# NVlabs/neuralrgbd

Hardware: AMD Instinct MI355X
Metric: depth frames/sec @256x192x64cand, 5-view window; warp-kernel HBM GB/s vs peak (higher is better)
Workload: dtype f32; 1 GPU; plane-sweep grid 256x192x64cand (image 1024x768); config_id=B, depth_candidates=64, views=5, streams_per_gpu=1, streams_total=1, parallelism=replicas x1 (independent video streams)

## Files before the change

### include/nrgbd.h

```cpp
#ifndef NRGBD_H
#define NRGBD_H

#ifdef __cplusplus
extern "C" {
#endif

#define NRGBD_OK             0
#define NRGBD_E_NULL        -1
#define NRGBD_E_SHAPE       -2
#define NRGBD_E_ALIGN       -3
#define NRGBD_E_ARG         -4

#define NRGBD_DIST_L2        0
#define NRGBD_DIST_L1        1

#define NRGBD_MAX_D        256
#define NRGBD_MAX_V         16

#define NRGBD_INTERFACE_VERSION "0.10"
const char* nrgbd_version(void);
const char* nrgbd_strerror(int code);

int nrgbd_homography_terms(const float* K, const float* R, long r_view_stride, long r_row_stride,
                           const float* t, long t_view_stride, long t_elem_stride, float* KR, float* Kt,
// ... 167 lines not shown
int nrgbd_conv_wino_dw4_workspace(int N, int H, int W, int Cout, size_t* bytes);
int nrgbd_conv_wino_dw4_f32(const float* x, const float* x_ss, int x_relu, float x_unit, const float* w_wino, float* y, float* stats,
                            void* workspace, size_t workspace_bytes, int N, int H, int W, int Cin, int Cout, void* stream);
int nrgbd_conv_wino_dw_unit_f32(const float* x, const float* x_ss, float x_unit, const float* w_wino, float* y, float* stats,
                                int N, int H, int W, int Cin, int Cout, void* stream);

int nrgbd_conv2d_rnet_f32(const float* x, const float* w_packed, const float* bias, int out_lrelu, float* y,
                          int ldy, int ycoff, int cout_valid, int mode, int pa, int pb,
                          int N, int H, int W, int Cin, int Cout, void* stream);
int nrgbd_rnet_pack(const float* dpv_log, const float* feat, int feat_planar, float* out, int D, int Cf, long P,
                    void* stream);

int nrgbd_conv2d_taps_f32(const float* x, const float* x_ss, int x_relu, const float* w_packed, float* y, float* stats,
                          int N, int H, int W, int Cin, int Cout, int taps, int in_stride, void* stream);
int nrgbd_space_to_depth2(const float* x, int nchw, float* y, int N, int C, int H, int W, int Cp, void* stream);
int nrgbd_conv2d_wgrad_workgroups(int N, int H, int W, int Cin, int Cout);
int nrgbd_conv2d_wgrad_f32(const float* x, const float* gy, float* partial, float* dw, int N, int H, int W, int Cin, int Cout,
                           int dilation, void* stream);
int nrgbd_conv2d_workgroups(int N, int H, int W);
int nrgbd_conv_pack_weights(const float* w, float* w_packed, int Cin, int Cout, int taps, void* stream);
int nrgbd_conv2d_3x3_f32(const float* x, const float* x_ss, int x_relu,
                         const float* res, const float* res_ss, int res_relu,
                         float* materialized, const float* w_packed, const float* bias, int out_lrelu,
                         float* y, float* stats, int N, int H, int W, int Cin, int Cout, int dilation,
                         void* stream);
int nrgbd_bn_finalize(const float* stats, int num_workgroups, int C, long count,
                      const float* gamma, const float* beta, float eps, float momentum,
                      float* running_mean, float* running_var, float* scale_shift, unsigned int* collapse_count, long long* batches_tracked, void* stream);
int nrgbd_bn_small_stats(int nseg, const float* const* x, const long* rows, int C, const float* const* gamma, const float* const* beta,
                     const float* eps, const float* momentum, float* const* running_mean, float* const* running_var,
// ... 62 lines not shown
```

### neuralrgbd_amd/_lib.py

```python
import ctypes
import os

_HERE = os.path.dirname(os.path.abspath(__file__))
LIB_PATH = os.path.join(_HERE, "csrc", "libnrgbd_hip.so")

_c = ctypes
_P = _c.c_void_p
_F = _c.c_float
_I = _c.c_int
_L = _c.c_long
_D = _c.c_double
_Z = _c.c_size_t

GATHER_MAX_V = 6
DEPTH_MAX_THRESHOLDS = 512
DEPTH_EVAL_MAX_SETS = 8
DGF_TILE = (16, 64)


class WindowSlots(ctypes.Structure):
    _fields_ = [("idx", _I * (GATHER_MAX_V + 1))]


SIGNATURES = {
# ... 59 lines not shown
    "nrgbd_conv3d_wgrad_ranges": (_I, []),
    "nrgbd_conv3d_wgrad_f32": (_I, [_P, _P, _P, _P, _I, _I, _I, _I, _P]),
    "nrgbd_bn3d_finalize": (_I, [_P, _I, _L, _P, _P, _F, _F, _P, _P, _P, _P, _P, _P]),
    "nrgbd_bn2d_partial_floats": (_I, [_I]),
    "nrgbd_bn2d_train_act": (_I, [_P, _P, _P, _F, _I, _P, _P, _P, _P, _I, _I, _L, _P]),
    "nrgbd_avgpool8": (_I, [_P, _P, _I, _I, _I, _P]),
    "nrgbd_conv2d_few_f32": (_I, [_P, _I, _P, _P, _I, _P, _I, _I, _I, _I, _I, _I, _I, _P]),
    "nrgbd_avgpool_cl": (_I, [_P, _P, _I, _I, _I, _I, _I, _P]),
    "nrgbd_scatter_channels": (_I, [_P, _L, _L, _L, _I, _I, _I, _P, _I, _I, _I, _L, _P]),
    "nrgbd_bias_act_nchw": (_I, [_P, _P, _F, _I, _I, _L, _P]),
    "nrgbd_conv2d_workgroups": (_I, [_I, _I, _I]),
    "nrgbd_conv2d_wgrad_workgroups": (_I, [_I, _I, _I, _I, _I]),
    "nrgbd_conv2d_wgrad_f32": (_I, [_P, _P, _P, _P, _I, _I, _I, _I, _I, _I, _P]),
    "nrgbd_conv2d_taps_f32": (_I, [_P, _P, _I, _P, _P, _P, _I, _I, _I, _I, _I, _I, _I, _P]),
    "nrgbd_space_to_depth2": (_I, [_P, _I, _P, _I, _I, _I, _I, _I, _P]),
    "nrgbd_conv_pack_weights": (_I, [_P, _P, _I, _I, _I, _P]),
    "nrgbd_conv2d_3x3_f32": (_I, [_P, _P, _I, _P, _P, _I, _P, _P, _P, _I, _P, _P, _I, _I, _I, _I, _I, _I, _P]),
    "nrgbd_conv2d_rnet_f32": (_I, [_P, _P, _P, _I, _P, _I, _I, _I, _I, _I, _I, _I, _I, _I, _I, _I, _P]),
    "nrgbd_rnet_pack": (_I, [_P, _P, _I, _P, _I, _I, _L, _P]),
    "nrgbd_bn_finalize": (_I, [_P, _I, _I, _L, _P, _P, _F, _F, _P, _P, _P, _P, _P, _P]),
    "nrgbd_logsoftmax_rows": (_I, [_P, _P, _L, _I, _P]),
    "nrgbd_logsoftmax_d_bwd": (_I, [_P, _P, _F, _P, _I, _L, _P]),
    "nrgbd_logsoftmax_rows_bwd": (_I, [_P, _P, _P, _L, _I, _P]),
    "nrgbd_nll_workgroups": (_I, [_L]),
    "nrgbd_nll_fwd": (_I, [_P, _P, _L, _I, _L, _I, _P, _P, _P]),
    "nrgbd_nll_bwd": (_I, [_P, _L, _P, _P, _P, _I, _L, _I, _P]),
    "nrgbd_adam_step": (_I, [_P, _P, _P, _P, _P, _P, _I, _D, _D, _D, _D, _D, _I, _P]),
    "nrgbd_grad_norm_workspace": (_L, [_P, _I]),
    "nrgbd_grad_norm": (_I, [_P, _P, _I, _D, _P, _Z, _P, _P, _P]),
    "nrgbd_scale_tensors": (_I, [_P, _P, _I, _P, _P]),
# ... 51 lines not shown
```

### neuralrgbd_amd/csrc/conv2d.hip

```cpp
#include <cstdlib>

#include "conv_tile.hpp"

namespace nrgbd {

constexpr int kT2 = 16;

struct Conv2dArgs {
    const float* x;
    const float* x_ss;
    const float* res;
    const float* res_ss;
    float* mat;
    const float* wp;
    const float* bias;
    float* y;
    float* stats;
    int x_relu, res_relu, out_lrelu;
    int N, H, W, Cin;
    int xcd;
    int ldy;
    int ycoff;
    int cout_valid;
    int up;
// ... 247 lines not shown
        }
        if (khalf == 0) {
#pragma unroll
            for (int f = 0; f < NF; ++f) {
                red[wv * (2 * COUT) + f * 32 + i] = s1[f];
                red[wv * (2 * COUT) + COUT + f * 32 + i] = s2[f];
            }
        }
        __syncthreads();
        if (tid < 2 * COUT)
            a.stats[(size_t)tile_id * (2 * COUT) + tid] =
                (red[tid] + red[2 * COUT + tid]) + (red[4 * COUT + tid] + red[6 * COUT + tid]);
    }
}

__global__ void conv_pack_weights_kernel(const float* __restrict__ w, float* __restrict__ wp, int Cin, int Cout, int taps) {
    const int ncblk = Cin / kCB, G4 = kCB / 8, nf = Cout / 32;
    const long total = (long)taps * Cin * Cout;
    const long idx = (long)blockIdx.x * 256 + threadIdx.x;
    if (idx >= total) return;
    long t = idx;
    const int e = t & 3; t >>= 2;
    const int ln = t & 63; t >>= 6;
    const int nfrag = t % nf; t /= nf;
    const int g = t % G4; t /= G4;
    const int cblk = t % ncblk; const int tap = (int)(t / ncblk);
    const int cout = nfrag * 32 + (ln & 31);
    const int cin = cblk * kCB + (ln >> 5) * (kCB / 2) + g * 4 + e;
    wp[idx] = w[((size_t)cout * Cin + cin) * taps + tap];
}
// ... 37 lines not shown
        v.x = __builtin_fmaf(v.x, ss[0], ss[1]); v.y = __builtin_fmaf(v.y, ss[2], ss[3]);
        v.z = __builtin_fmaf(v.z, ss[4], ss[5]); v.w = __builtin_fmaf(v.w, ss[6], ss[7]);
    }
    if (x_relu) { v.x = fmaxf(v.x, 0.f); v.y = fmaxf(v.y, 0.f); v.z = fmaxf(v.z, 0.f); v.w = fmaxf(v.w, 0.f); }
    if (res) {
        f32x4 r = *reinterpret_cast<const f32x4*>(res + p * C + c);
        if (res_ss) {
            const float* ss = res_ss + 2 * c;
            r.x = __builtin_fmaf(r.x, ss[0], ss[1]); r.y = __builtin_fmaf(r.y, ss[2], ss[3]);
            r.z = __builtin_fmaf(r.z, ss[4], ss[5]); r.w = __builtin_fmaf(r.w, ss[6], ss[7]);
        }
        if (res_relu) { r.x = fmaxf(r.x, 0.f); r.y = fmaxf(r.y, 0.f); r.z = fmaxf(r.z, 0.f); r.w = fmaxf(r.w, 0.f); }
        v = v + r;
    }
    *reinterpret_cast<f32x4*>(y + p * ldy + c) = v;
}

__global__ __launch_bounds__(256) void bn_finalize_kernel(const float* __restrict__ stats, int nwg, int C, double count,
                                                          const float* __restrict__ gamma, const float* __restrict__ beta,
                                                          float eps, float momentum, float* __restrict__ running_mean,
                                                          float* __restrict__ running_var, float* __restrict__ ss, unsigned int* __restrict__ collapse_count, long long* __restrict__ batches_tracked) {
    __shared__ double sh[2][256];
    const int c = blockIdx.x, tid = threadIdx.x;
    double s1 = 0.0, s2 = 0.0;
    for (int g = tid; g < nwg; g += 256) {
        s1 += (double)stats[(size_t)g * 2 * C + c];
        s2 += (double)stats[(size_t)g * 2 * C + C + c];
    }
    sh[0][tid] = s1; sh[1][tid] = s2;
    __syncthreads();
// ... 123 lines not shown
    if ((long)N * H * W * Cin * in_stride * in_stride >= (1L << 32)) return NRGBD_E_SHAPE;
    Conv2dArgs a{x, x_ss, nullptr, nullptr, nullptr, w_packed, nullptr, y, stats, x_relu, 0, 0, N, H, W, Cin,
                 0, Cout, 0, Cout, 0, 0, 0, nullptr, in_stride};
    const int nwg = ceil_div(W, kT2) * ceil_div(H, kT2) * N;
    hipStream_t st = (hipStream_t)stream;
    if (taps == 1) {
        if (Cout == 32) launch_conv2d_taps<32, 1>(a, nwg, st);
        else if (Cout == 64) launch_conv2d_taps<64, 1>(a, nwg, st);
        else if (Cout == 128) launch_conv2d_taps<128, 1>(a, nwg, st);
        else return NRGBD_E_SHAPE;
    } else {
        if (Cout == 32) launch_conv2d_taps<32, 4>(a, nwg, st);
        else if (Cout == 64) launch_conv2d_taps<64, 4>(a, nwg, st);
        else return NRGBD_E_SHAPE;
    }
    NRGBD_CHECK_LAUNCH();
    return NRGBD_OK;
}

extern "C" int nrgbd_conv2d_workgroups(int N, int H, int W) {
    using namespace nrgbd;
    if (N <= 0 || H <= 0 || W <= 0) return NRGBD_E_SHAPE;
    return ceil_div(W, kT2) * ceil_div(H, kT2) * N;
}

extern "C" int nrgbd_conv_pack_weights(const float* w, float* wp, int Cin, int Cout, int taps, void* stream) {
    using namespace nrgbd;
    if (!w || !wp) return NRGBD_E_NULL;
    if (Cin <= 0 || Cin % kCB || Cout <= 0 || Cout % 32 || (taps != 9 && taps != 27 && taps != 4 && taps != 1)) return NRGBD_E_SHAPE;
    const long total = (long)taps * Cin * Cout;
// ... 112 lines not shown
    return NRGBD_OK;
}

extern "C" int nrgbd_nhwc_act(const float* x, const float* x_ss, int x_relu, const float* res, const float* res_ss,
                              int res_relu, float* y, long P, int C, int ldy, void* stream) {
    using namespace nrgbd;
    if (!x || !y) return NRGBD_E_NULL;
    if (P <= 0 || C < 4 || (C & 3) || ldy < C || (ldy & 3)) return NRGBD_E_SHAPE;
    const long total = P * (C >> 2);
    hipLaunchKernelGGL(nhwc_act_kernel, dim3((unsigned)((total + 255) / 256)), dim3(256), 0, (hipStream_t)stream, x, x_ss,
                       x_relu, res, res_ss, res_relu, y, P, C, ldy);
    NRGBD_CHECK_LAUNCH();
    return NRGBD_OK;
}

extern "C" int nrgbd_bn_finalize(const float* stats, int num_workgroups, int C, long count, const float* gamma,
                                 const float* beta, float eps, float momentum, float* running_mean, float* running_var,
                                 float* scale_shift, unsigned int* collapse_count, long long* batches_tracked, void* stream) {
    using namespace nrgbd;
    if (!stats || !gamma || !beta || !scale_shift) return NRGBD_E_NULL;
    if (num_workgroups <= 0 || count <= 0 || C <= 0) return NRGBD_E_SHAPE;
    if ((running_mean == nullptr) != (running_var == nullptr)) return NRGBD_E_NULL;
    hipLaunchKernelGGL(bn_finalize_kernel, dim3(C), dim3(256), 0, (hipStream_t)stream, stats, num_workgroups, C,
                       (double)count, gamma, beta, eps, momentum, running_mean, running_var, scale_shift, collapse_count, batches_tracked);
    NRGBD_CHECK_LAUNCH();
    return NRGBD_OK;
}
```

### neuralrgbd_amd/csrc/warpvol.hip

```cpp
#include "common.hpp"

namespace nrgbd {

struct WarpVolArgs {
    const float* src; long sv, sc, sy, sx;
    const float* ref; long rc, ry, rx;
    const float* KR; const float* Kt; const float* rays; const float* d_candi;
    const float* bv_cur; const float* bv_pred;
    float* out;
    float cx, cy;
    int align, V, Cs, D, h, w;
    int channels_last;
    int ld;
};

__global__ __launch_bounds__(256) void warp_volume_kernel(const WarpVolArgs a) {
    const size_t hw = (size_t)a.h * a.w;
    const size_t p = (size_t)blockIdx.x * 256 + threadIdx.x;
    const int k = blockIdx.y;
    if (p >= hw) return;
    const int y = (int)(p / a.w), x = (int)(p - (size_t)y * a.w);
    const float rx = a.rays[p], ry = a.rays[hw + p], rz = a.rays[2 * hw + p];
    const float d = a.d_candi[k];
    const float wf = (float)a.w, hf = (float)a.h;
// ... 14 lines not shown
            o[(size_t)(v * a.Cs + c) * plane] = lerp4(pl[onw], pl[one], pl[osw], pl[ose], b);
        }
    }
    int ch = a.V * a.Cs;
    if (a.ref) {
        for (int c = 0; c < a.Cs; ++c) o[(size_t)(ch + c) * plane] = a.ref[c * a.rc + y * a.ry + x * a.rx];
        ch += a.Cs;
    }
    if (a.bv_cur) o[(size_t)ch * plane] = a.bv_cur[(size_t)k * hw + p] - a.bv_pred[(size_t)k * hw + p];
    if (a.channels_last)
        for (int c = n_ch; c < ld; ++c) o[c] = 0.f;
}

template <bool ALIGN>
__global__ __launch_bounds__(256) void warp_volume_cl16_kernel(const WarpVolArgs a, float rcx, float rcy) {
    const size_t hw = (size_t)a.h * a.w;
    const size_t p = (size_t)blockIdx.x * 256 + threadIdx.x;
    const int k = blockIdx.y;
    if (p >= hw) return;
    const int y = (int)(p / a.w), x = (int)(p - (size_t)y * a.w);
    const float rx = a.rays[p], ry = a.rays[hw + p], rz = a.rays[2 * hw + p];
    const float d = a.d_candi[k];
    const float wf = (float)a.w, hf = (float)a.h;
    float o[16];
#pragma unroll
    for (int v = 0; v < 4; ++v) {
        const SweepTerm st = make_sweep_term(a.KR + 9 * v, a.Kt + 3 * v, rx, ry, rz);
        float ix, iy;
        sweep_sample_pos_fast<ALIGN>(st, d, a.cx, a.cy, rcx, rcy, wf, hf, ix, iy);
        const Bilinear b = bilinear_zeros(ix, iy, a.w, a.h);
        const float* s = a.src + v * a.sv;
        const float4 A = *reinterpret_cast<const float4*>(s + b.y0 * a.sy + b.x0 * a.sx);
        const float4 B = *reinterpret_cast<const float4*>(s + b.y0 * a.sy + b.x1 * a.sx);
        const float4 C = *reinterpret_cast<const float4*>(s + b.y1 * a.sy + b.x0 * a.sx);
        const float4 Dd = *reinterpret_cast<const float4*>(s + b.y1 * a.sy + b.x1 * a.sx);
        o[3 * v + 0] = lerp4(A.x, B.x, C.x, Dd.x, b);
        o[3 * v + 1] = lerp4(A.y, B.y, C.y, Dd.y, b);
        o[3 * v + 2] = lerp4(A.z, B.z, C.z, Dd.z, b);
    }
    const float4 r = *reinterpret_cast<const float4*>(a.ref + y * a.ry + x * a.rx);
    o[12] = r.x; o[13] = r.y; o[14] = r.z;
    o[15] = a.bv_cur[(size_t)k * hw + p] - a.bv_pred[(size_t)k * hw + p];
    float4* dst = reinterpret_cast<float4*>(a.out + ((size_t)k * hw + p) * 16);
#pragma unroll
    for (int q = 0; q < 4; ++q) dst[q] = make_float4(o[4 * q], o[4 * q + 1], o[4 * q + 2], o[4 * q + 3]);
}

template <int V, int CP, bool ALIGN>
__global__ __launch_bounds__(256) void warp_volume_cl_kernel(const WarpVolArgs a, float rcx, float rcy) {
    constexpr int C = 3 * V + 4;
    static_assert(CP % 4 == 0 && CP >= C, "padded voxel holds the assembly in whole 16-byte words");
    const size_t hw = (size_t)a.h * a.w;
    const size_t p = (size_t)blockIdx.x * 256 + threadIdx.x;
    const int k = blockIdx.y;
    if (p >= hw) return;
    const int y = (int)(p / a.w), x = (int)(p - (size_t)y * a.w);
    const float rx = a.rays[p], ry = a.rays[hw + p], rz = a.rays[2 * hw + p];
    const float d = a.d_candi[k];
    const float wf = (float)a.w, hf = (float)a.h;
    float o[CP];
// ... 86 lines not shown
```

### neuralrgbd_amd/nets.py

```python
import math

import numpy as np
import torch
import torch.nn as nn
import torch.nn.functional as F


def _conv_bn2d(cin, cout, k, stride, pad, dilation, track=False):
    p = dilation if dilation > 1 else pad
    return nn.Sequential(
        nn.Conv2d(cin, cout, k, stride=stride, padding=p, dilation=dilation, bias=False),
        nn.BatchNorm2d(cout, track_running_stats=track),
    )


def _conv_bn3d(cin, cout):
    return nn.Sequential(nn.Conv3d(cin, cout, 3, stride=1, padding=1, bias=False), nn.BatchNorm3d(cout))


def _conv_lrelu(cin, cout):
    return nn.Sequential(nn.Conv2d(cin, cout, 3, stride=1, padding=1, bias=True), nn.LeakyReLU())


def _deconv_lrelu(cin, cout):
# ... 5 lines not shown
        if isinstance(m, (nn.Conv2d, nn.Conv3d)):
            fan = int(np.prod(m.kernel_size)) * m.out_channels
            m.weight.data.normal_(0, math.sqrt(2.0 / fan))
        elif isinstance(m, (nn.BatchNorm2d, nn.BatchNorm3d)):
            m.weight.data.fill_(1)
            m.bias.data.zero_()



def _no_kernel(what):
    from ._lib import NrgbdError
    return NrgbdError("no hand-written kernel for " + what)


class _Act(object):
    __slots__ = ("z", "ss", "relu", "r", "r_ss", "r_relu")

    def __init__(self, z, ss=None, relu=False, r=None, r_ss=None, r_relu=False):
        self.z, self.ss, self.relu, self.r, self.r_ss, self.r_relu = z, ss, relu, r, r_ss, r_relu


_PACKERS = {
    "taps": lambda ops, w: ops.conv_pack_weights(w),
    "s2": lambda ops, w: ops.conv_s2_pack(w),
    "pc": lambda ops, w: ops.conv_wino_pack32(w) if w.shape[0] == 32 and w.dim() == 4 else ops.conv_wino_pack(w),
    "dw": lambda ops, w: ops.conv_wino_dw_pack(w),
    "dw4": lambda ops, w: ops.conv_wino_dw4_pack(w),
    "direct": lambda ops, w: ops.conv3d_pack_weights(w),
    "cout1": lambda ops, w: w[0].reshape(w.shape[1], 27).t().contiguous(),
}


def padded_channels(c):
    return -(-int(c) // 16) * 16


def pad_input_channels(w, cin):
    if cin == w.shape[1]:
        return w
    return torch.cat((w, w.new_zeros((w.shape[0], cin - w.shape[1]) + tuple(w.shape[2:]))), dim=1)


def _packed(owner, conv, kind, mult=1.0, cin=None):
    from . import ops
    cache = owner.__dict__.setdefault("_wp_cache", {})
# ... 214 lines not shown
                and ops.conv_wino_supported(a.z.shape[0], a.z.shape[1], a.z.shape[2], conv.in_channels, conv.out_channels, 1))
        if wino:
            z, st, mat = ops.conv_wino(a.z, _packed(self, conv, "pc"), conv.out_channels, 1, d, x_ss=a.ss, x_relu=a.relu,
                                       res=a.r, res_ss=a.r_ss, res_relu=a.r_relu, materialize=materialize,
                                       want_stats=_needs_stats(bn))
        elif mfma:
            z, st, mat = ops.conv2d(a.z, _packed(self, conv, "taps"), conv.out_channels, d, x_ss=a.ss, x_relu=a.relu,
                                    res=a.r, res_ss=a.r_ss, res_relu=a.r_relu, materialize=materialize,
                                    want_stats=_needs_stats(bn))
        else:
            mat = a.z if (a.ss is None and a.r is None and not a.relu) else \
                ops.nhwc_act(a.z, a.ss, a.relu, a.r, a.r_ss, a.r_relu)
            s2 = (conv.kernel_size == (3, 3) and conv.stride == (2, 2) and conv.padding == (1, 1) and d == 1
                  and mat.shape[1] % 2 == 0 and mat.shape[2] % 2 == 0 and conv.out_channels in (32, 64))
            if s2:
                z, st = ops.conv2d_taps(ops.space_to_depth2(mat), _packed(self, conv, "s2"), conv.out_channels, 4,
                                        want_stats=_needs_stats(bn))
            else:
                raise _no_kernel("feature CNN layer %d -> %d, kernel %s, stride %s, dilation %d on a %d x %d map" % (
                    conv.in_channels, conv.out_channels, tuple(conv.kernel_size), tuple(conv.stride), d, mat.shape[1], mat.shape[2]))
        count = z.shape[0] * z.shape[1] * z.shape[2]
        return _Act(z, _bn_scale_shift(bn, st, count, "cm" if wino else "rows"), relu), mat

    def _pointwise_cl(self, conv, m, stride=1, want_stats=False):
        from . import ops
        N, H, W, C = m.shape
        if C % 16 != 0 or conv.out_channels not in (32, 64, 128) or H % stride or W % stride:
            raise _no_kernel("1x1 layer %d -> %d, stride %d on a %d x %d map" % (C, conv.out_channels, stride, H, W))
        return ops.conv2d_taps(m.contiguous(), _packed(self, conv, "taps"), conv.out_channels, 1, want_stats=want_stats, stride=stride)

    def _pointwise_bn_cl(self, seq, m, stride=1):
        conv, bn = seq[0], seq[1]
        z, st = self._pointwise_cl(conv, m, stride, want_stats=_needs_stats(bn))
        return _Act(z, _bn_scale_shift(bn, st, z.shape[0] * z.shape[1] * z.shape[2]), False)

    def _block_cl(self, blk, a):
        y1, m = self._conv_bn_cl(blk.conv1[0], a, relu=True, materialize=True)
        y2, _ = self._conv_bn_cl(blk.conv2, y1, relu=False)
        if blk.downsample is None:
            return _Act(y2.z, y2.ss, False, r=m)
        sk = self._pointwise_bn_cl(blk.downsample, m, blk.downsample[0].stride[0])
        return _Act(y2.z, y2.ss, False, r=sk.z, r_ss=sk.ss)

    def fused_ok(self, x):
        return x.is_cuda and not torch.is_grad_enabled() and x.dtype == torch.float32

    def forward_channels_last(self, x):
        from . import ops
        conv, bn = self.firstconv[0]
        if x.shape[2] % 4 or x.shape[3] % 4:
            raise _no_kernel("image %d x %d: the plane-sweep grid is the image / 4 (models/basic.py:254-263), both sides must be multiples of 4"
                             % (x.shape[2], x.shape[3]))
        z, st = ops.conv2d_taps(ops.space_to_depth2(x.contiguous(), nchw=True), _packed(self, conv, "s2"), conv.out_channels, 4,
                                want_stats=_needs_stats(bn))
        a = _Act(z, _bn_scale_shift(bn, st, z.numel() // z.shape[-1]), True)
        for i in (2, 4):
            a, _ = self._conv_bn_cl(self.firstconv[i], a, relu=True)
        for blk in self.layer1:
            a = self._block_cl(blk, a)
        half = ops.nhwc_act(a.z, a.ss, a.relu, a.r, a.r_ss, a.r_relu)
        a = _Act(half)
        for blk in self.layer2:
            a = self._block_cl(blk, a)
        quarter = None
        for k, blk in enumerate(self.layer3):
            y1, m = self._conv_bn_cl(blk.conv1[0], a, relu=True, materialize=True)
            if k == 0:
                quarter = m
            y2, _ = self._conv_bn_cl(blk.conv2, y1, relu=False)
            if blk.downsample is None:
                a = _Act(y2.z, y2.ss, False, r=m)
            else:
                sk = self._pointwise_bn_cl(blk.downsample, m, blk.downsample[0].stride[0])
                a = _Act(y2.z, y2.ss, False, r=sk.z, r_ss=sk.ss)
        for blk in self.layer4:
            a = self._block_cl(blk, a)
# ... 8 lines not shown
            pools = {8: p8, 16: p16, 32: p32, 64: ops.avgpool_cl(p32, 2)}
        else:
            pools = {k: ops.avgpool_cl(deep, k) for k in self.SPP_WINDOWS}
        zs, norms = [], []
        for i in (4, 3, 2, 1):
            branch = getattr(self, "branch%d" % i)
            z, _ = self._pointwise_cl(branch[1][0], pools[self.SPP_WINDOWS[i - 1]])
            zs.append(z)
            norms.append(branch[1][1])
        sss = _bn_scale_shift_small(norms, zs)
        cat = ops.spp_concat(quarter, deep, list(zip(zs, sss)))
        y, _ = self._conv_bn_cl(self.lastconv[0], _Act(cat), relu=True)
        head = self.lastconv[2]
        if head.out_channels not in (32, 64, 128):
            raise _no_kernel("feature_dim %d (1x1 head): 32, 64 or 128" % head.out_channels)
        feat, _ = ops.conv2d_taps(y.z, _packed(self, head, "taps"), head.out_channels, 1, x_ss=y.ss, x_relu=True, want_stats=False)
        return half, feat

    def forward(self, x):
        if x.is_cuda:
            x = x.contiguous(memory_format=torch.channels_last)
        stem = x
        for i in (0, 2, 4):
            stem = _conv_bn_act(stem, self.firstconv[i], relu=True)
        half = self.layer1(stem)
        quarter = self.layer2(half)
        deep = self.layer4(self.layer3(quarter))
        size = deep.shape[2:]
        pools = self._spp_pools(deep)
        pyramid = []
        for i in (4, 3, 2, 1):
# ... 463 lines not shown
```

### neuralrgbd_amd/ops.py

```python
import ctypes

import numpy as np
import torch

from . import _lib

DIST = {"L2": 0, "L1": 1}
GENERATION = {None: 0, "auto": 0, "gather": 1, "lds": 2, "quad": 3}


def _need(t, name, shape=None, strided=False):
    if not isinstance(t, torch.Tensor):
        raise TypeError("%s must be a torch.Tensor" % name)
    if not t.is_cuda:
        raise _lib.NrgbdError("%s is on %s: the plane-sweep path runs on the GPU only "
                              "(no CPU fallback)" % (name, t.device))
    if t.dtype != torch.float32:
        raise TypeError("%s must be float32, got %s" % (name, t.dtype))
    if shape is not None and tuple(t.shape) != tuple(shape):
        raise ValueError("%s has shape %s, expected %s" % (name, tuple(t.shape), tuple(shape)))
    return t if (strided or t.is_contiguous()) else t.contiguous()


def _p(t):
# ... 766 lines not shown
    x = _need(x, "x")
    N, H, W, Cin = x.shape
    if stride != 1:
        if taps != 1 or H % stride or W % stride:
            raise ValueError("conv2d_taps: a stride needs taps = 1 and sides that are multiples of it")
        H, W = H // stride, W // stride
    y = torch.empty((N, H, W, cout), dtype=torch.float32, device=x.device)
    stats = torch.empty((conv2d_workgroups(N, H, W), 2 * cout), dtype=torch.float32, device=x.device) if want_stats else None
    with torch.cuda.device(x.device):
        rc = _lib.load().nrgbd_conv2d_taps_f32(_p(x), _p(x_ss), int(x_relu), _p(w_packed), _p(y), _p(stats), N, H, W, Cin,
                                                int(cout), int(taps), int(stride), _stream(x))
    _lib.check(rc, "nrgbd_conv2d_taps_f32")
    return y, stats


def conv2d_wgrad(x, gy, dilation=1):
    x = _need(x, "x")
    N, H, W, Cin = x.shape
    gy = _need(gy, "gy")
    Cout = gy.shape[-1]
    if tuple(gy.shape[:3]) != (N, H, W):
        raise ValueError("conv2d_wgrad: gy %s does not match x %s" % (tuple(gy.shape), tuple(x.shape)))
    lib = _lib.load()
    nwg = int(lib.nrgbd_conv2d_wgrad_workgroups(N, H, W, Cin, Cout))
    _lib.check(min(nwg, 0), "nrgbd_conv2d_wgrad_workgroups")
    blocks = -(-Cout // 64) * -(-Cin // 64)
    partial = torch.empty(blocks * nwg * 9 * 64 * 64, dtype=torch.float32, device=x.device)
    dw = torch.empty((Cout, Cin, 3, 3), dtype=torch.float32, device=x.device)
    with torch.cuda.device(x.device):
        rc = lib.nrgbd_conv2d_wgrad_f32(_p(x), _p(gy), _p(partial), _p(dw), N, H, W, Cin, Cout, int(dilation), _stream(x))
# ... 313 lines not shown
def nhwc_act(x, x_ss=None, x_relu=False, res=None, res_ss=None, res_relu=False, out=None, ldy=None):
    x = _need(x, "x")
    C = x.shape[-1]
    P = x.numel() // C
    if res is not None:
        res = _need(res, "res", x.shape)
    if out is None:
        out, ldy = torch.empty_like(x), C
    elif ldy is None:
        raise ValueError("nhwc_act: out needs its pixel stride ldy")
    with torch.cuda.device(x.device):
        rc = _lib.load().nrgbd_nhwc_act(_p(x), _p(x_ss), int(x_relu), _p(res), _p(res_ss), int(res_relu), _p(out), P, C,
                                         int(ldy), _stream(x))
    _lib.check(rc, "nrgbd_nhwc_act")
    return out


def bn2d_train_act(x, gamma, beta, eps, relu=False, residual=None, inplace=True, want_mean_var=False):
    x = _need(x, "x")
    N, C, H, W = x.shape
    if residual is not None:
        residual = _need(residual, "residual", x.shape)
    y = x if inplace else torch.empty_like(x)
    partial = torch.empty(int(_lib.load().nrgbd_bn2d_partial_floats(C)), dtype=torch.float32, device=x.device)
    mv = torch.empty((C, 2), dtype=torch.float32, device=x.device) if want_mean_var else None
    with torch.cuda.device(x.device):
        rc = _lib.load().nrgbd_bn2d_train_act(_p(x), _p(gamma), _p(beta), float(eps), int(bool(relu)), _p(residual),
                                               _p(y), _p(partial), _p(mv), N, C, H * W, _stream(x))
    _lib.check(rc, "nrgbd_bn2d_train_act")
    return y, mv
# ... 248 lines not shown
```

Before: 30.50 frames/s.

## Add specialized 1x1, RGB stride-2 conv kernels and fused act+space-to-depth

Adds a dedicated MFMA 1x1 convolution kernel with an LDS-staged coalesced epilogue, a first-layer RGB stride-2 conv that reads the planar image directly instead of running space_to_depth first, and a fused activation kernel that also emits the space-to-depth copy for the next stride-2 layer. The cost-volume gather output is also restaged through shared memory so global stores are coalesced. Together these cut kernel launches and intermediate HBM round trips in the feature CNN. They add code and new shape-specific paths that may have edge-case bugs.

```diff
diff --git a/include/nrgbd.h b/include/nrgbd.h
--- a/include/nrgbd.h
+++ b/include/nrgbd.h
@@ -205,6 +205,11 @@
 int nrgbd_conv2d_taps_f32(const float* x, const float* x_ss, int x_relu, const float* w_packed, float* y, float* stats,
                           int N, int H, int W, int Cin, int Cout, int taps, int in_stride, void* stream);
 int nrgbd_space_to_depth2(const float* x, int nchw, float* y, int N, int C, int H, int W, int Cp, void* stream);
+int nrgbd_nhwc_act_s2d(const float* x, const float* x_ss, int x_relu, const float* res, const float* res_ss, int res_relu,
+                       float* y, float* y2, int N, int C, int H, int W, int Cp, void* stream);
+int nrgbd_conv2d_rgb_s2_f32(const float* img, const float* w_packed, float* y, float* stats, int N, int H, int W, void* stream);
+int nrgbd_conv1x1_f32(const float* x, const float* x_ss, int x_relu, const float* w_packed, const float* bias, float* y,
+                      float* stats, int N, int H, int W, int Cin, int Cout, int in_stride, void* stream);
 int nrgbd_conv2d_wgrad_workgroups(int N, int H, int W, int Cin, int Cout);
 int nrgbd_conv2d_wgrad_f32(const float* x, const float* gy, float* partial, float* dw, int N, int H, int W, int Cin, int Cout,
                            int dilation, void* stream);
diff --git a/neuralrgbd_amd/_lib.py b/neuralrgbd_amd/_lib.py
--- a/neuralrgbd_amd/_lib.py
+++ b/neuralrgbd_amd/_lib.py
@@ -97,6 +97,9 @@
     "nrgbd_conv2d_wgrad_f32": (_I, [_P, _P, _P, _P, _I, _I, _I, _I, _I, _I, _P]),
     "nrgbd_conv2d_taps_f32": (_I, [_P, _P, _I, _P, _P, _P, _I, _I, _I, _I, _I, _I, _I, _P]),
     "nrgbd_space_to_depth2": (_I, [_P, _I, _P, _I, _I, _I, _I, _I, _P]),
+    "nrgbd_nhwc_act_s2d": (_I, [_P, _P, _I, _P, _P, _I, _P, _P, _I, _I, _I, _I, _I, _P]),
+    "nrgbd_conv2d_rgb_s2_f32": (_I, [_P, _P, _P, _P, _I, _I, _I, _P]),
+    "nrgbd_conv1x1_f32": (_I, [_P, _P, _I, _P, _P, _P, _P, _I, _I, _I, _I, _I, _I, _P]),
     "nrgbd_conv_pack_weights": (_I, [_P, _P, _I, _I, _I, _P]),
     "nrgbd_conv2d_3x3_f32": (_I, [_P, _P, _I, _P, _P, _I, _P, _P, _P, _I, _P, _P, _I, _I, _I, _I, _I, _I, _P]),
     "nrgbd_conv2d_rnet_f32": (_I, [_P, _P, _P, _I, _P, _I, _I, _I, _I, _I, _I, _I, _I, _I, _I, _I, _P]),
diff --git a/neuralrgbd_amd/csrc/conv2d.hip b/neuralrgbd_amd/csrc/conv2d.hip
--- a/neuralrgbd_amd/csrc/conv2d.hip
+++ b/neuralrgbd_amd/csrc/conv2d.hip
@@ -285,6 +285,234 @@
     }
 }
 
+constexpr int kStagePitch = 36, kStageWave = 32 * kStagePitch + 32;
+
+template <int COUT>
+__device__ __forceinline__ void tile_epilogue(const Conv2dArgs& a, f32x16 (&acc)[2][COUT / 32], float* red, float* stage, int n, int y0,
+                                              int x0, int tile_id) {
+    constexpr int NF = COUT / 32;
+    const int tid = threadIdx.x, lane = tid & 63, wv = tid >> 6, i = lane & 31, khalf = lane >> 5, wy = wv * 4;
+    float s1[NF], s2[NF], bs[NF];
+#pragma unroll
+    for (int f = 0; f < NF; ++f) { s1[f] = 0.f; s2[f] = 0.f; bs[f] = a.bias ? a.bias[f * 32 + i] : 0.f; }
+    float* st = stage + wv * kStageWave;
+    const int px8 = lane >> 3, cq = (lane & 7) * 4;
+#pragma unroll
+    for (int m = 0; m < 2; ++m) {
+        bool own_ok[2];
+        float* wr[2];
+        bool line_ok[2];
+        float* line[2];
+#pragma unroll
+        for (int c = 0; c < 2; ++c) {
+            own_ok[c] = y0 + wy + 2 * m + (khalf ^ c) < a.H;
+            wr[c] = st + (khalf ^ c) * (16 * kStagePitch + 32) + i;
+            const int gy = y0 + wy + 2 * m + c;
+            line_ok[c] = gy < a.H;
+            line[c] = a.y + (((size_t)n * a.H + (line_ok[c] ? gy : 0)) * a.W + x0 + px8) * COUT + cq;
+        }
+#pragma unroll
+        for (int f = 0; f < NF; ++f) {
+#pragma unroll
+            for (int r = 0; r < 16; ++r) {
+                const int c = (r >= 4 && r < 12) ? 1 : 0;
+                const float z = acc[m][f][r] + bs[f];
+                wr[c][r * kStagePitch] = z;
+                if (own_ok[c] && x0 + r < a.W) {
+                    s1[f] += z;
+                    s2[f] = __builtin_fmaf(z, z, s2[f]);
+                }
+            }
+            __builtin_amdgcn_fence(__ATOMIC_RELEASE, "wavefront");
+            __builtin_amdgcn_wave_barrier();
+            __builtin_amdgcn_fence(__ATOMIC_ACQUIRE, "wavefront");
+#pragma unroll
+            for (int j = 0; j < 4; ++j) {
+                const int c = j >> 1, x = px8 + 8 * (j & 1);
+                const f32x4 v = *reinterpret_cast<const f32x4*>(st + c * (16 * kStagePitch + 32) + x * kStagePitch + cq);
+                if (line_ok[c] && x0 + x < a.W) *reinterpret_cast<f32x4*>(line[c] + (8 * (j & 1)) * COUT + f * 32) = v;
+            }
+            __builtin_amdgcn_fence(__ATOMIC_RELEASE, "wavefront");
+            __builtin_amdgcn_wave_barrier();
+            __builtin_amdgcn_fence(__ATOMIC_ACQUIRE, "wavefront");
+        }
+    }
+    if (a.stats) {
+#pragma unroll
+        for (int f = 0; f < NF; ++f) {
+            s1[f] += __shfl_xor(s1[f], 32, 64);
+            s2[f] += __shfl_xor(s2[f], 32, 64);
+        }
+        if (khalf == 0) {
+#pragma unroll
+            for (int f = 0; f < NF; ++f) {
+                red[wv * (2 * COUT) + f * 32 + i] = s1[f];
+                red[wv * (2 * COUT) + COUT + f * 32 + i] = s2[f];
+            }
+        }
+        __syncthreads();
+        if (tid < 2 * COUT)
+            a.stats[(size_t)tile_id * (2 * COUT) + tid] =
+                (red[tid] + red[2 * COUT + tid]) + (red[4 * COUT + tid] + red[6 * COUT + tid]);
+    }
+}
+
+template <int COUT, int NCB, bool SS>
+__global__ __launch_bounds__(256, 2) void conv1x1_mfma_kernel(const Conv2dArgs a) {
+    constexpr int NF = COUT / 32, G4 = kCB / 8, Cin = NCB * kCB;
+    constexpr int AD = (COUT > 64 && SS) ? 1 : 2;
+    __shared__ float red[4 * 2 * COUT];
+    __shared__ __attribute__((aligned(16))) float stage[4 * kStageWave];
+
+    const int tid = threadIdx.x, lane = tid & 63, wv = tid >> 6;
+    const int tiles_x = (a.W + kT2 - 1) / kT2, tiles_y = (a.H + kT2 - 1) / kT2;
+    int t = xcd_tile(blockIdx.x, gridDim.x, a.xcd);
+    const int tile_id = t;
+    const int tx = t % tiles_x; t /= tiles_x;
+    const int ty = t % tiles_y; const int n = t / tiles_y;
+    const int x0 = tx * kT2, y0 = ty * kT2;
+
+    const int i = lane & 31, khalf = lane >> 5;
+    int dy, px;
+    row_to_yx(i, dy, px);
+    const int wy = wv * 4;
+    const int xs = a.xs > 1 ? a.xs : 1;
+    const float* xp[2];
+#pragma unroll
+    for (int m = 0; m < 2; ++m) {
+        const int gy = y0 + wy + 2 * m + dy, gx = x0 + px;
+        const bool ok = gy < a.H && gx < a.W;
+        xp[m] = a.x + (ok ? (((size_t)n * (a.H * xs) + (size_t)gy * xs) * (a.W * xs) + (size_t)gx * xs) * Cin : (size_t)0) + khalf * 8;
+    }
+    const f32x4* wb = reinterpret_cast<const f32x4*>(a.wp) + lane;
+    const float* sp = SS ? a.x_ss + 2 * (khalf * 8) : nullptr;
+
+    f32x16 acc[2][NF];
+#pragma unroll
+    for (int m = 0; m < 2; ++m)
+#pragma unroll
+        for (int f = 0; f < NF; ++f)
+#pragma unroll
+            for (int e = 0; e < 16; ++e) acc[m][f][e] = 0.f;
+
+    constexpr int NS = NCB * G4, BD = AD;
+    f32x4 A[NCB][G4][2], B[NS][NF], S[SS ? NS : 1][2];
+    auto load_b = [&](int s) {
+#pragma unroll
+        for (int f = 0; f < NF; ++f) B[s][f] = wb[s * (NF * 64) + f * 64];
+        if constexpr (SS) {
+            const int ch = (s / G4) * kCB + (s % G4) * 4;
+            S[s][0] = *reinterpret_cast<const f32x4*>(sp + 2 * ch);
+            S[s][1] = *reinterpret_cast<const f32x4*>(sp + 2 * ch + 4);
+        }
+    };
+    auto load_a = [&](int c) {
+#pragma unroll
+        for (int g = 0; g < G4; ++g)
+#pragma unroll
+            for (int m = 0; m < 2; ++m) A[c][g][m] = *reinterpret_cast<const f32x4*>(xp[m] + c * kCB + g * 4);
+    };
+#pragma unroll
+    for (int s = 0; s < BD && s < NS; ++s) load_b(s);
+#pragma unroll
+    for (int c = 0; c < AD && c < NCB; ++c) load_a(c);
+#pragma unroll
+    for (int c = 0; c < NCB; ++c) {
+#pragma unroll
+        for (int g = 0; g < G4; ++g) {
+            __builtin_amdgcn_sched_barrier(0);
+            if (c * G4 + g + BD < NS) load_b(c * G4 + g + BD);
+            if (g == 0 && c + AD < NCB) load_a(c + AD);
+#pragma unroll
+            for (int m = 0; m < 2; ++m) {
+                f32x4 v = A[c][g][m];
+                if constexpr (SS) {
+                    const f32x4 s0 = S[c * G4 + g][0], s1 = S[c * G4 + g][1];
+                    v.x = __builtin_fmaf(v.x, s0.x, s0.y); v.y = __builtin_fmaf(v.y, s0.z, s0.w);
+                    v.z = __builtin_fmaf(v.z, s1.x, s1.y); v.w = __builtin_fmaf(v.w, s1.z, s1.w);
+                }
+                if (a.x_relu) { v.x = fmaxf(v.x, 0.f); v.y = fmaxf(v.y, 0.f); v.z = fmaxf(v.z, 0.f); v.w = fmaxf(v.w, 0.f); }
+                A[c][g][m] = v;
+            }
+#pragma unroll
+            for (int e = 0; e < 4; ++e)
+#pragma unroll
+                for (int m = 0; m < 2; ++m)
+#pragma unroll
+                    for (int f = 0; f < NF; ++f)
+                        acc[m][f] = __builtin_amdgcn_mfma_f32_32x32x2f32(A[c][g][m][e], B[c * G4 + g][f][e], acc[m][f], 0, 0, 0);
+        }
+    }
+
+    tile_epilogue<COUT>(a, acc, red, stage, n, y0, x0, tile_id);
+}
+
+template <int COUT, int NCB>
+static void launch_conv1x1(const Conv2dArgs& a, int nwg, hipStream_t st) {
+    if (a.x_ss) hipLaunchKernelGGL((conv1x1_mfma_kernel<COUT, NCB, true>), dim3(nwg), dim3(256), 0, st, a);
+    else        hipLaunchKernelGGL((conv1x1_mfma_kernel<COUT, NCB, false>), dim3(nwg), dim3(256), 0, st, a);
+}
+
+__global__ __launch_bounds__(256, 3) void conv_rgb_s2_mfma_kernel(const Conv2dArgs a) {
+    constexpr int COUT = 32, NS = 8;
+    __shared__ float red[4 * 2 * COUT];
+    __shared__ __attribute__((aligned(16))) float stage[4 * kStageWave];
+    const int tid = threadIdx.x, lane = tid & 63, wv = tid >> 6;
+    const int tiles_x = (a.W + kT2 - 1) / kT2, tiles_y = (a.H + kT2 - 1) / kT2;
+    int t = blockIdx.x;
+    const int tile_id = t;
+    const int tx = t % tiles_x; t /= tiles_x;
+    const int ty = t % tiles_y; const int n = t / tiles_y;
+    const int x0 = tx * kT2, y0 = ty * kT2;
+    const int i = lane & 31, khalf = lane >> 5;
+    int dy, px;
+    row_to_yx(i, dy, px);
+    const int wy = wv * 4;
+    const int Hi = 2 * a.H, Wi = 2 * a.W;
+    const float* img = a.x + (size_t)n * 3 * Hi * Wi;
+
+    int eo[2][4];
+#pragma unroll
+    for (int g = 0; g < 2; ++g)
+#pragma unroll
+        for (int e = 0; e < 4; ++e) {
+            const int ch = khalf * 8 + g * 4 + e, ph = (ch * 11) >> 5, c = ch - 3 * ph;
+            eo[g][e] = ch < 12 ? (c * Hi + (ph >> 1)) * Wi + (ph & 1) : -1;
+        }
+    const f32x4* wb = reinterpret_cast<const f32x4*>(a.wp) + lane;
+    f32x4 A[NS][2], B[NS];
+#pragma unroll
+    for (int s = 0; s < NS; ++s) {
+        B[s] = wb[s * 64];
+        const int tap = s >> 1, g = s & 1;
+#pragma unroll
+        for (int m = 0; m < 2; ++m) {
+            const int Y = y0 + wy + 2 * m + dy + (tap >> 1) - 1, X = x0 + px + (tap & 1) - 1;
+            const bool in = Y >= 0 && Y < a.H && X >= 0 && X < a.W;
+            const int base = 2 * Y * Wi + 2 * X;
+#pragma unroll
+            for (int e = 0; e < 4; ++e) {
+                const bool ok = in && eo[g][e] >= 0;
+                const float v = img[ok ? base + eo[g][e] : 0];
+                A[s][m][e] = ok ? v : 0.f;
+            }
+        }
+    }
+    f32x16 acc[2][1];
+#pragma unroll
+    for (int m = 0; m < 2; ++m)
+#pragma unroll
+        for (int e = 0; e < 16; ++e) acc[m][0][e] = 0.f;
+#pragma unroll
+    for (int s = 0; s < NS; ++s)
+#pragma unroll
+        for (int e = 0; e < 4; ++e)
+#pragma unroll
+            for (int m = 0; m < 2; ++m)
+                acc[m][0] = __builtin_amdgcn_mfma_f32_32x32x2f32(A[s][m][e], B[s][e], acc[m][0], 0, 0, 0);
+    tile_epilogue<COUT>(a, acc, red, stage, n, y0, x0, tile_id);
+}
+
 __global__ void conv_pack_weights_kernel(const float* __restrict__ w, float* __restrict__ wp, int Cin, int Cout, int taps) {
     const int ncblk = Cin / kCB, G4 = kCB / 8, nf = Cout / 32;
     const long total = (long)taps * Cin * Cout;
@@ -352,6 +580,45 @@
         v = v + r;
     }
     *reinterpret_cast<f32x4*>(y + p * ldy + c) = v;
+}
+
+__global__ __launch_bounds__(256) void nhwc_act_s2d_kernel(const float* __restrict__ x, const float* __restrict__ x_ss, int x_relu,
+                                                           const float* __restrict__ res, const float* __restrict__ res_ss,
+                                                           int res_relu, float* __restrict__ y, float* __restrict__ y2, int N, int C,
+                                                           int H, int W, int Cp) {
+    const int Ho = H >> 1, Wo = W >> 1, q4 = Cp >> 2;
+    const long total = (long)N * Ho * Wo * q4;
+    const long idx = (long)blockIdx.x * 256 + threadIdx.x;
+    if (idx >= total) return;
+    const int cp = (int)(idx % q4) * 4;
+    long t = idx / q4;
+    const int xo = (int)(t % Wo); t /= Wo;
+    const int yo = (int)(t % Ho);
+    const int n = (int)(t / Ho);
+    f32x4 v = {0.f, 0.f, 0.f, 0.f};
+    if (cp < 4 * C) {
+        const int ph = cp / C, c = cp - ph * C;
+        const size_t o = (((size_t)n * H + 2 * yo + (ph >> 1)) * W + 2 * xo + (ph & 1)) * C + c;
+        v = *reinterpret_cast<const f32x4*>(x + o);
+        if (x_ss) {
+            const float* ss = x_ss + 2 * c;
+            v.x = __builtin_fmaf(v.x, ss[0], ss[1]); v.y = __builtin_fmaf(v.y, ss[2], ss[3]);
+            v.z = __builtin_fmaf(v.z, ss[4], ss[5]); v.w = __builtin_fmaf(v.w, ss[6], ss[7]);
+        }
+        if (x_relu) { v.x = fmaxf(v.x, 0.f); v.y = fmaxf(v.y, 0.f); v.z = fmaxf(v.z, 0.f); v.w = fmaxf(v.w, 0.f); }
+        if (res) {
+            f32x4 r = *reinterpret_cast<const f32x4*>(res + o);
+            if (res_ss) {
+                const float* ss = res_ss + 2 * c;
+                r.x = __builtin_fmaf(r.x, ss[0], ss[1]); r.y = __builtin_fmaf(r.y, ss[2], ss[3]);
+                r.z = __builtin_fmaf(r.z, ss[4], ss[5]); r.w = __builtin_fmaf(r.w, ss[6], ss[7]);
+            }
+            if (res_relu) { r.x = fmaxf(r.x, 0.f); r.y = fmaxf(r.y, 0.f); r.z = fmaxf(r.z, 0.f); r.w = fmaxf(r.w, 0.f); }
+            v = v + r;
+        }
+        *reinterpret_cast<f32x4*>(y + o) = v;
+    }
+    *reinterpret_cast<f32x4*>(y2 + idx * 4) = v;
 }
 
 __global__ __launch_bounds__(256) void bn_finalize_kernel(const float* __restrict__ stats, int nwg, int C, double count,
@@ -505,6 +772,42 @@
         else if (Cout == 64) launch_conv2d_taps<64, 4>(a, nwg, st);
         else return NRGBD_E_SHAPE;
     }
+    NRGBD_CHECK_LAUNCH();
+    return NRGBD_OK;
+}
+
+extern "C" int nrgbd_conv1x1_f32(const float* x, const float* x_ss, int x_relu, const float* w_packed, const float* bias, float* y,
+                                 float* stats, int N, int H, int W, int Cin, int Cout, int in_stride, void* stream) {
+    using namespace nrgbd;
+    if (!x || !w_packed || !y) return NRGBD_E_NULL;
+    if (N <= 0 || H <= 0 || W <= 0 || Cin <= 0) return NRGBD_E_SHAPE;
+    if (in_stride < 1 || in_stride > 8) return NRGBD_E_ARG;
+    if ((long)N * H * W * Cin * in_stride * in_stride >= (1L << 32)) return NRGBD_E_SHAPE;
+    Conv2dArgs a{x, x_ss, nullptr, nullptr, nullptr, w_packed, bias, y, stats, x_relu, 0, 0, N, H, W, Cin,
+                 0, Cout, 0, Cout, 0, 0, 0, nullptr, in_stride};
+    const int nwg = ceil_div(W, kT2) * ceil_div(H, kT2) * N;
+    hipStream_t st = (hipStream_t)stream;
+    if (Cout == 64 && Cin == 32) launch_conv1x1<64, 2>(a, nwg, st);
+    else if (Cout == 64 && Cin == 64) launch_conv1x1<64, 4>(a, nwg, st);
+    else if (Cout == 64 && Cin == 128) launch_conv1x1<64, 8>(a, nwg, st);
+    else if (Cout == 128 && Cin == 32) launch_conv1x1<128, 2>(a, nwg, st);
+    else if (Cout == 128 && Cin == 64) launch_conv1x1<128, 4>(a, nwg, st);
+    else if (Cout == 128 && Cin == 128) launch_conv1x1<128, 8>(a, nwg, st);
+    else return NRGBD_E_SHAPE;
+    NRGBD_CHECK_LAUNCH();
+    return NRGBD_OK;
+}
+
+extern "C" int nrgbd_conv2d_rgb_s2_f32(const float* img, const float* w_packed, float* y, float* stats, int N, int H, int W,
+                                      void* stream) {
+    using namespace nrgbd;
+    if (!img || !w_packed || !y) return NRGBD_E_NULL;
+    if (N <= 0 || H <= 0 || W <= 0) return NRGBD_E_SHAPE;
+    if (12L * H * W >= (1L << 31) || (long)N * H * W * 32 >= (1L << 32)) return NRGBD_E_SHAPE;
+    Conv2dArgs a{img, nullptr, nullptr, nullptr, nullptr, w_packed, nullptr, y, stats, 0, 0, 0, N, H, W, 16,
+                 0, 32, 0, 32, 0, 0, 0, nullptr, 0};
+    const int nwg = ceil_div(W, kT2) * ceil_div(H, kT2) * N;
+    hipLaunchKernelGGL(conv_rgb_s2_mfma_kernel, dim3(nwg), dim3(256), 0, (hipStream_t)stream, a);
     NRGBD_CHECK_LAUNCH();
     return NRGBD_OK;
 }
@@ -647,6 +950,20 @@
     return NRGBD_OK;
 }
 
+extern "C" int nrgbd_nhwc_act_s2d(const float* x, const float* x_ss, int x_relu, const float* res, const float* res_ss, int res_relu,
+                                  float* y, float* y2, int N, int C, int H, int W, int Cp, void* stream) {
+    using namespace nrgbd;
+    if (!x || !y || !y2) return NRGBD_E_NULL;
+    if (N <= 0 || C < 4 || (C & 3) || H <= 0 || W <= 0 || (H & 1) || (W & 1) || Cp < 4 * C || (Cp & 3)) return NRGBD_E_SHAPE;
+    if ((reinterpret_cast<uintptr_t>(x) | reinterpret_cast<uintptr_t>(res) | reinterpret_cast<uintptr_t>(y) | reinterpret_cast<uintptr_t>(y2)) & 15)
+        return NRGBD_E_ALIGN;
+    const long total = (long)N * (H / 2) * (W / 2) * (Cp / 4);
+    hipLaunchKernelGGL(nhwc_act_s2d_kernel, dim3((unsigned)((total + 255) / 256)), dim3(256), 0, (hipStream_t)stream, x, x_ss, x_relu,
+                       res, res_ss, res_relu, y, y2, N, C, H, W, Cp);
+    NRGBD_CHECK_LAUNCH();
+    return NRGBD_OK;
+}
+
 extern "C" int nrgbd_bn_finalize(const float* stats, int num_workgroups, int C, long count, const float* gamma,
                                  const float* beta, float eps, float momentum, float* running_mean, float* running_var,
                                  float* scale_shift, unsigned int* collapse_count, long long* batches_tracked, void* stream) {
diff --git a/neuralrgbd_amd/csrc/warpvol.hip b/neuralrgbd_amd/csrc/warpvol.hip
--- a/neuralrgbd_amd/csrc/warpvol.hip
+++ b/neuralrgbd_amd/csrc/warpvol.hip
@@ -52,10 +52,11 @@
 
 template <bool ALIGN>
 __global__ __launch_bounds__(256) void warp_volume_cl16_kernel(const WarpVolArgs a, float rcx, float rcy) {
+    __shared__ __attribute__((aligned(16))) float stage[4][64 * 20];
     const size_t hw = (size_t)a.h * a.w;
-    const size_t p = (size_t)blockIdx.x * 256 + threadIdx.x;
+    const size_t pl = (size_t)blockIdx.x * 256 + threadIdx.x;
     const int k = blockIdx.y;
-    if (p >= hw) return;
+    const size_t p = pl < hw ? pl : hw - 1;
     const int y = (int)(p / a.w), x = (int)(p - (size_t)y * a.w);
     const float rx = a.rays[p], ry = a.rays[hw + p], rz = a.rays[2 * hw + p];
     const float d = a.d_candi[k];
@@ -79,9 +80,19 @@
     const float4 r = *reinterpret_cast<const float4*>(a.ref + y * a.ry + x * a.rx);
     o[12] = r.x; o[13] = r.y; o[14] = r.z;
     o[15] = a.bv_cur[(size_t)k * hw + p] - a.bv_pred[(size_t)k * hw + p];
-    float4* dst = reinterpret_cast<float4*>(a.out + ((size_t)k * hw + p) * 16);
+    const int lane = threadIdx.x & 63, wv = threadIdx.x >> 6;
+    float* sw = stage[wv];
 #pragma unroll
-    for (int q = 0; q < 4; ++q) dst[q] = make_float4(o[4 * q], o[4 * q + 1], o[4 * q + 2], o[4 * q + 3]);
+    for (int q = 0; q < 4; ++q)
+        *reinterpret_cast<float4*>(sw + lane * 20 + 4 * q) = make_float4(o[4 * q], o[4 * q + 1], o[4 * q + 2], o[4 * q + 3]);
+    __syncthreads();
+    const size_t w0 = (size_t)blockIdx.x * 256 + wv * 64;
+#pragma unroll
+    for (int q = 0; q < 4; ++q) {
+        const int j = (lane >> 2) + 16 * q, wd = lane & 3;
+        const float4 v = *reinterpret_cast<const float4*>(sw + j * 20 + 4 * wd);
+        if (w0 + j < hw) *reinterpret_cast<float4*>(a.out + ((size_t)k * hw + w0 + j) * 16 + 4 * wd) = v;
+    }
 }
 
 template <int V, int CP, bool ALIGN>
diff --git a/neuralrgbd_amd/nets.py b/neuralrgbd_amd/nets.py
--- a/neuralrgbd_amd/nets.py
+++ b/neuralrgbd_amd/nets.py
@@ -43,10 +43,11 @@
 
 
 class _Act(object):
-    __slots__ = ("z", "ss", "relu", "r", "r_ss", "r_relu")
-
-    def __init__(self, z, ss=None, relu=False, r=None, r_ss=None, r_relu=False):
+    __slots__ = ("z", "ss", "relu", "r", "r_ss", "r_relu", "s2d")
+
+    def __init__(self, z, ss=None, relu=False, r=None, r_ss=None, r_relu=False, s2d=None):
         self.z, self.ss, self.relu, self.r, self.r_ss, self.r_relu = z, ss, relu, r, r_ss, r_relu
+        self.s2d = s2d
 
 
 _PACKERS = {
@@ -58,6 +59,10 @@
     "direct": lambda ops, w: ops.conv3d_pack_weights(w),
     "cout1": lambda ops, w: w[0].reshape(w.shape[1], 27).t().contiguous(),
 }
+
+
+def _pointwise_shape(cin, cout):
+    return cin in (32, 64, 128) and cout in (64, 128)
 
 
 def padded_channels(c):
@@ -302,8 +307,8 @@
             s2 = (conv.kernel_size == (3, 3) and conv.stride == (2, 2) and conv.padding == (1, 1) and d == 1
                   and mat.shape[1] % 2 == 0 and mat.shape[2] % 2 == 0 and conv.out_channels in (32, 64))
             if s2:
-                z, st = ops.conv2d_taps(ops.space_to_depth2(mat), _packed(self, conv, "s2"), conv.out_channels, 4,
-                                        want_stats=_needs_stats(bn))
+                x2 = a.s2d if (mat is a.z and a.s2d is not None) else ops.space_to_depth2(mat)
+                z, st = ops.conv2d_taps(x2, _packed(self, conv, "s2"), conv.out_channels, 4, want_stats=_needs_stats(bn))
             else:
                 raise _no_kernel("feature CNN layer %d -> %d, kernel %s, stride %s, dilation %d on a %d x %d map" % (
                     conv.in_channels, conv.out_channels, tuple(conv.kernel_size), tuple(conv.stride), d, mat.shape[1], mat.shape[2]))
@@ -315,6 +320,8 @@
         N, H, W, C = m.shape
         if C % 16 != 0 or conv.out_channels not in (32, 64, 128) or H % stride or W % stride:
             raise _no_kernel("1x1 layer %d -> %d, stride %d on a %d x %d map" % (C, conv.out_channels, stride, H, W))
+        if _pointwise_shape(C, conv.out_channels):
+            return ops.conv1x1(m.contiguous(), _packed(self, conv, "taps"), conv.out_channels, want_stats=want_stats, stride=stride)
         return ops.conv2d_taps(m.contiguous(), _packed(self, conv, "taps"), conv.out_channels, 1, want_stats=want_stats, stride=stride)
 
     def _pointwise_bn_cl(self, seq, m, stride=1):
@@ -339,15 +346,22 @@
         if x.shape[2] % 4 or x.shape[3] % 4:
             raise _no_kernel("image %d x %d: the plane-sweep grid is the image / 4 (models/basic.py:254-263), both sides must be multiples of 4"
                              % (x.shape[2], x.shape[3]))
-        z, st = ops.conv2d_taps(ops.space_to_depth2(x.contiguous(), nchw=True), _packed(self, conv, "s2"), conv.out_channels, 4,
-                                want_stats=_needs_stats(bn))
+        if conv.out_channels == 32:
+            z, st = ops.conv2d_rgb_s2(x.contiguous(), _packed(self, conv, "s2"), want_stats=_needs_stats(bn))
+        else:
+            z, st = ops.conv2d_taps(ops.space_to_depth2(x.contiguous(), nchw=True), _packed(self, conv, "s2"), conv.out_channels, 4,
+                                    want_stats=_needs_stats(bn))
         a = _Act(z, _bn_scale_shift(bn, st, z.numel() // z.shape[-1]), True)
         for i in (2, 4):
             a, _ = self._conv_bn_cl(self.firstconv[i], a, relu=True)
         for blk in self.layer1:
             a = self._block_cl(blk, a)
-        half = ops.nhwc_act(a.z, a.ss, a.relu, a.r, a.r_ss, a.r_relu)
-        a = _Act(half)
+        c2 = self.layer2[0].conv1[0][0]
+        if c2.kernel_size == (3, 3) and c2.stride == (2, 2) and c2.out_channels in (32, 64):
+            half, half2 = ops.nhwc_act_s2d(a.z, a.ss, a.relu, a.r, a.r_ss, a.r_relu)
+        else:
+            half, half2 = ops.nhwc_act(a.z, a.ss, a.relu, a.r, a.r_ss, a.r_relu), None
+        a = _Act(half, s2d=half2)
         for blk in self.layer2:
             a = self._block_cl(blk, a)
         quarter = None
@@ -386,7 +400,10 @@
         head = self.lastconv[2]
         if head.out_channels not in (32, 64, 128):
             raise _no_kernel("feature_dim %d (1x1 head): 32, 64 or 128" % head.out_channels)
-        feat, _ = ops.conv2d_taps(y.z, _packed(self, head, "taps"), head.out_channels, 1, x_ss=y.ss, x_relu=True, want_stats=False)
+        if _pointwise_shape(y.z.shape[-1], head.out_channels):
+            feat, _ = ops.conv1x1(y.z, _packed(self, head, "taps"), head.out_channels, x_ss=y.ss, x_relu=True, want_stats=False)
+        else:
+            feat, _ = ops.conv2d_taps(y.z, _packed(self, head, "taps"), head.out_channels, 1, x_ss=y.ss, x_relu=True, want_stats=False)
         return half, feat
 
     def forward(self, x):
diff --git a/neuralrgbd_amd/ops.py b/neuralrgbd_amd/ops.py
--- a/neuralrgbd_amd/ops.py
+++ b/neuralrgbd_amd/ops.py
@@ -804,6 +804,36 @@
     return y, stats
 
 
+def conv1x1(x, w_packed, cout, x_ss=None, x_relu=False, want_stats=True, stride=1, bias=None):
+    x = _need(x, "x")
+    N, H, W, Cin = x.shape
+    if stride != 1:
+        if H % stride or W % stride:
+            raise ValueError("conv1x1: a stride needs sides that are multiples of it")
+        H, W = H // stride, W // stride
+    y = torch.empty((N, H, W, cout), dtype=torch.float32, device=x.device)
+    stats = torch.empty((conv2d_workgroups(N, H, W), 2 * cout), dtype=torch.float32, device=x.device) if want_stats else None
+    with torch.cuda.device(x.device):
+        rc = _lib.load().nrgbd_conv1x1_f32(_p(x), _p(x_ss), int(x_relu), _p(w_packed), _p(bias), _p(y), _p(stats), N, H, W, Cin,
+                                            int(cout), int(stride), _stream(x))
+    _lib.check(rc, "nrgbd_conv1x1_f32")
+    return y, stats
+
+
+def conv2d_rgb_s2(img, w_packed, want_stats=True):
+    img = _need(img, "img")
+    N, C, H, W = img.shape
+    if C != 3 or H % 2 or W % 2:
+        raise ValueError("conv2d_rgb_s2: a planar RGB image with even sides, got %s" % (tuple(img.shape),))
+    H, W = H // 2, W // 2
+    y = torch.empty((N, H, W, 32), dtype=torch.float32, device=img.device)
+    stats = torch.empty((conv2d_workgroups(N, H, W), 64), dtype=torch.float32, device=img.device) if want_stats else None
+    with torch.cuda.device(img.device):
+        rc = _lib.load().nrgbd_conv2d_rgb_s2_f32(_p(img), _p(w_packed), _p(y), _p(stats), N, H, W, _stream(img))
+    _lib.check(rc, "nrgbd_conv2d_rgb_s2_f32")
+    return y, stats
+
+
 def conv2d_wgrad(x, gy, dilation=1):
     x = _need(x, "x")
     N, H, W, Cin = x.shape
@@ -1147,6 +1177,21 @@
                                          int(ldy), _stream(x))
     _lib.check(rc, "nrgbd_nhwc_act")
     return out
+
+
+def nhwc_act_s2d(x, x_ss=None, x_relu=False, res=None, res_ss=None, res_relu=False, cp=None):
+    x = _need(x, "x")
+    N, H, W, C = x.shape
+    if res is not None:
+        res = _need(res, "res", x.shape)
+    cp = cp or -(-4 * C // 16) * 16
+    y = torch.empty_like(x)
+    y2 = torch.empty((N, H // 2, W // 2, cp), dtype=torch.float32, device=x.device)
+    with torch.cuda.device(x.device):
+        rc = _lib.load().nrgbd_nhwc_act_s2d(_p(x), _p(x_ss), int(x_relu), _p(res), _p(res_ss), int(res_relu), _p(y), _p(y2),
+                                             N, C, H, W, cp, _stream(x))
+    _lib.check(rc, "nrgbd_nhwc_act_s2d")
+    return y, y2
 
 
 def bn2d_train_act(x, gamma, beta, eps, relu=False, residual=None, inplace=True, want_mean_var=False):
```

Result: no change. 30.61 frames/s (median of 6 runs) (+0.3%).
